# anyboby/Constrained-Model-Based-Policy-Optimization

Measured on AMD Instinct MI355X. Metric: imagined env-steps/sec (ensemble rollout) + CPO update ms, higher is better.
Workload: dtype f32; 1 GPU; AntSafe-v2 imagined rollout: E=7 x (37->512->512->60) swish ensemble, 5 elites, 3+3 critics 128x128, tanh policy 128x128, B=100000 branches/GPU, maxroll 35 (34 steps), fixed-horizon mode, reset->sample*->finish_all_paths->get(); rollout_mode=schedule, branches_per_gpu=100000, branches_total=100000, horizon=34, task=AntSafe-v2

## Files before the change

constrained-model-based-policy-optimization_amd/csrc/ens_h3.hip:

```cpp
#include "common.h"
#include "ens_mlp_internal.h"
#include "f16_split.h"

#include <type_traits>

namespace {

constexpr int kThreadsH = 512;
constexpr int kWavesH = 8;
constexpr int HIDH = 512;

template <int RT>
struct Geo {
  static constexpr int ROWS = 32 * RT;
  static constexpr int NTC = 8 / RT;
  static constexpr int CK = 32 * NTC;
  static constexpr int NCH = HIDH / CK;
  static constexpr int SLC = CK / 32;
  static constexpr int CSTR = CK + 8;
  static constexpr int TPR = kThreadsH / ROWS;
  static constexpr int KPT = 64 / TPR;
  static constexpr int DH = RT == 4 ? 2 : 4;
  static constexpr int NPH = (2 * SLC) % DH == 0 ? 1 : DH;
  static constexpr int CBUF_BYTES = 2 * ROWS * CSTR * 2;
  static constexpr bool W0_LDS = RT == 4;
};

constexpr int PBUF_BYTES = kWavesH * 2 * 16 * 64 * 4;
constexpr int SWS = 65;
constexpr int STG_BYTES = 32 * SWS * 4;
__host__ __device__ constexpr int ximg_bytes(int S0, int RT) { return 2 * 32 * RT * (16 * S0 + 8) * 2; }
__host__ __device__ constexpr int w0buf_bytes(int S0, int RT) { return RT == 4 ? 2 * S0 * 2 * 1024 : 0; }
__host__ __device__ constexpr int off_const(int S0, int RT) {
  const int cb = RT == 4 ? Geo<4>::CBUF_BYTES : (RT == 2 ? Geo<2>::CBUF_BYTES : Geo<1>::CBUF_BYTES);
  const int a = 2 * cb + ximg_bytes(S0, RT) + 2 * w0buf_bytes(S0, RT), b = 2 * PBUF_BYTES + 2 * STG_BYTES;
  return ((a > b ? a : b) + 15) / 16 * 16;
}
constexpr int CONST_FLOATS = 2 * HIDH + 2 * 128 + 6 * 128 + 2 * 64;
__host__ __device__ constexpr int lds_bytes(int S0, int RT) { return off_const(S0, RT) + CONST_FLOATS * 4; }

#ifdef CMBPO_STAMPS
#define H3_STAMP(k)                                                         \
  do {                                                                      \
    __builtin_amdgcn_sched_barrier(0);                                      \
    const unsigned long long t_now = __builtin_amdgcn_s_memtime();          \
    __builtin_amdgcn_s_waitcnt(0xC07F);                                     \
    t_acc[k] += t_now - t_last;                                             \
    t_last = t_now;                                                         \
    __builtin_amdgcn_sched_barrier(0);                                      \
  } while (0)
#else
#define H3_STAMP(k) do { } while (0)
#endif

__global__ void h3_stats_kernel(const float *blob, size_t off0, size_t off1, size_t off2, size_t offb0, size_t offb1, size_t offb2,
                                int kg0, int o_tiles, int hidden, float *stats) {
  const int e = blockIdx.x, l = blockIdx.y, tid = threadIdx.x;
  const int tiles = l == 2 ? o_tiles : hidden / 32, kg = l == 0 ? kg0 : hidden / 8;
  const size_t woff = l == 0 ? off0 : (l == 1 ? off1 : off2), boff = l == 0 ? offb0 : (l == 1 ? offb1 : offb2);
  const float *w = blob + woff + (size_t)e * tiles * kg * 256;
  const float *b = blob + boff + (size_t)e * tiles * 32;
  float wmax = 0.0f, l1 = 0.0f, bmax = 0.0f;
  if (tid < tiles * 32) {
    const int tile = tid >> 5, r = tid & 31;
    for (int g = 0; g < kg; ++g)
      for (int h = 0; h < 2; ++h) {
        const f32x4 v = *reinterpret_cast<const f32x4 *>(w + (((size_t)tile * kg + g) * 64 + h * 32 + r) * 4);
        for (int s = 0; s < 4; ++s) { const float a = fabsf(v[s]); wmax = fmaxf(wmax, a); l1 += a; }
      }
    bmax = fabsf(b[tid]);
  }
  __shared__ float red[3][kThreadsH];
  red[0][tid] = wmax; red[1][tid] = l1; red[2][tid] = bmax;
  __syncthreads();
  for (int st = kThreadsH / 2; st > 0; st >>= 1) {
    if (tid < st)
      for (int q = 0; q < 3; ++q) red[q][tid] = fmaxf(red[q][tid], red[q][tid + st]);
    __syncthreads();
  }
  if (tid == 0) {
    float *o = stats + (size_t)e * NSTAT + 4 * l;
    o[0] = pow2_lift(red[0][0]); o[1] = red[1][0]; o[2] = red[2][0]; o[3] = red[0][0];
  }
}

__global__ void h3_pack_kernel(const float *src, size_t src_stride, int kg, int src_tiles, f16x8 *dst, size_t dst_stride,
                               int n_tiles, int slabs, int members, const float *stats, int layer, int mode) {
  const long idx = (long)blockIdx.x * blockDim.x + threadIdx.x;
  const long per = (long)n_tiles * slabs * 64;
  if (idx >= per * members) return;
  const int e = (int)(idx / per);
  const int rem = (int)(idx - (long)e * per);
  const int lane = rem & 63, s = (rem >> 6) % slabs, tile = (rem >> 6) / slabs;
  const bool m16 = mode >= 2;
  const int n = m16 ? 16 * tile + (lane & 15) : 32 * tile + (lane & 31);
  const int r = n & 31, g = m16 ? lane >> 4 : lane >> 5;
  const float scale = stats[(size_t)e * NSTAT + 4 * layer];
  const float *sp = src + (size_t)e * src_stride;
  f16x8 p1, p2;
#pragma unroll
  for (int j = 0; j < 8; ++j) {
    int k;
    if (mode == 0) k = 16 * s + 8 * g + j;
    else if (mode == 1) {
      const int i = 8 * (s & 1) + j;
      k = 32 * (s >> 1) + (i & 3) + 8 * (i >> 2) + 4 * g;
    } else if (mode == 2) k = 32 * s + 8 * ((g & 1) * 2 + (g >> 1)) + j;
    else k = 32 * s + 16 * (j >> 2) + 4 * g + (j & 3);
    float v = 0.0f;
    if ((n >> 5) < src_tiles && (k >> 3) < kg) v = sp[(((size_t)(n >> 5) * kg + (k >> 3)) * 64 + ((k >> 2) & 1) * 32 + r) * 4 + (k & 3)];
    _Float16 q1, q2;
    split_h(v * scale, q1, q2);
    p1[j] = q1; p2[j] = q2;
  }
  f16x8 *d = dst + (size_t)e * dst_stride + ((size_t)tile * slabs + s) * 2 * 64 + lane;
  d[0] = p1; d[64] = p2;
}

template <int I, int N, class F>
__device__ __forceinline__ void static_for(F &&f) {
  if constexpr (I < N) {
    f(std::integral_constant<int, I>{});
    static_for<I + 1, N>(f);
  }
}


struct H3Args {
  MlpKernelArgs m;
  const f16x8 *w0, *w1, *w2;
  size_t w0_stride, w1_stride, w2_stride;
  const float *stats;
  int item0;
};

template <int S0, int OTP, int RT>
__global__ __launch_bounds__(kThreadsH, 2) void ens_h3_kernel(const H3Args a) {
  using G = Geo<RT>;
  constexpr int ROWSH = G::ROWS, NTC = G::NTC, CK = G::CK, NCH = G::NCH, SLC = G::SLC, CSTR = G::CSTR, TPR = G::TPR,
                KPT = G::KPT, DH = G::DH, NPH = G::NPH, CBUF_BYTES = G::CBUF_BYTES;
  constexpr int XSTR = 16 * S0 + 8;
  constexpr int NPASS = OTP / 2;
  constexpr int NUNIT = RT * NPASS;
  constexpr int O_PAD = 32 * OTP;
  constexpr int W0P = NTC * S0 * 2;
  const MlpKernelArgs &p = a.m;
  extern __shared__ f32x4 smem4[];
  char *smem = reinterpret_cast<char *>(smem4);
  _Float16 *cbuf = reinterpret_cast<_Float16 *>(smem);
  _Float16 *ximg = reinterpret_cast<_Float16 *>(smem + 2 * CBUF_BYTES);
  f16x8 *w0buf = reinterpret_cast<f16x8 *>(smem + 2 * CBUF_BYTES + ximg_bytes(S0, RT));
  f32x4 *pbuf = reinterpret_cast<f32x4 *>(smem);
  float *stg = reinterpret_cast<float *>(smem + 2 * PBUF_BYTES);
  float *cst = reinterpret_cast<float *>(smem + off_const(S0, RT));
  float *bias0 = cst, *bias1 = cst + HIDH, *hc_a = cst + 2 * HIDH, *hc_c = hc_a + 128;
  int *rowidx = reinterpret_cast<int *>(hc_c + 128);
  float *r_inv0 = reinterpret_cast<float *>(rowidx) + 128, *r_t1 = r_inv0 + 128, *r_inv1 = r_t1 + 128, *r_t2 = r_inv1 + 128,
        *r_inv2 = r_t2 + 128;
  float *in_mu_l = r_inv2 + 128, *in_sig_l = in_mu_l + 64;

  const int n_rows = p.n_rows_dev ? *p.n_rows_dev : p.n_rows;
  const int out = p.out_dim;
  if (threadIdx.x < 64) {
    const int k = threadIdx.x;
    in_mu_l[k] = (p.in_mu && k < p.in_dim) ? p.in_mu[k] : 0.0f;
    in_sig_l[k] = (p.in_mu && k < p.in_dim) ? 1.0f / p.in_sig[k] : 1.0f;
  }
  __syncthreads();

  float xpre[KPT];
  float bpre[2], b2pre = 0.0f;
  int rr_pre = -1;
  auto fetch_row = [&](int it, int tid) {
    const int xb = tid / TPR;
    const int e2 = it / p.tiles;
    const int rr = (it - e2 * p.tiles) * ROWSH + xb;
    const bool ok = it < p.n_items && rr < n_rows;
    int v = ok ? rr : 0;
    if (p.row_idx) v = p.row_idx[v];
    rr_pre = ok ? v : -1;
  };
  auto fetch_x = [&](int tid) {
    const int xc = tid % TPR;
    const int rr = rr_pre >= 0 ? rr_pre : 0;
    const float *orow = p.obs + (size_t)rr * p.obs_dim;
    const float *arow = p.act_dim > 0 ? p.act + (size_t)rr * p.act_dim - p.obs_dim : orow;
#pragma unroll
    for (int u = 0; u < KPT; ++u) {
      const int k = KPT * xc + u;
      const float *q = (k < p.obs_dim) ? orow + k : ((k < p.in_dim) ? arow + k : orow);
      xpre[u] = *q;
    }
  };
  auto fetch_bias = [&](int it, int tid) {
    const int e2 = (it < p.n_items) ? it / p.tiles : 0;
    bpre[0] = p.b0[(size_t)e2 * HIDH + tid];
    bpre[1] = p.b1[(size_t)e2 * HIDH + tid];
    const int ob = p.o_tiles * 32;
    b2pre = p.b2[(size_t)e2 * ob + (tid < ob ? tid : 0)];
  };
  fetch_row(a.item0 + blockIdx.x, threadIdx.x);
  fetch_x(threadIdx.x);
  fetch_bias(a.item0 + blockIdx.x, threadIdx.x);
#ifdef CMBPO_STAMPS
  unsigned long long t_acc[12] = {0, 0, 0, 0, 0, 0, 0, 0, 0, 0, 0, 0};
  unsigned long long t_last = __builtin_amdgcn_s_memtime();
  const unsigned long long t_rt0 = __builtin_amdgcn_s_memrealtime();
#endif

  for (int item = a.item0 + blockIdx.x; item < p.n_items; item += gridDim.x) {
    int tid = threadIdx.x;
    asm volatile("v_mov_b32 %0, %0" : "+v"(tid));
    const int lane = tid & 63, wave = __builtin_amdgcn_readfirstlane(tid >> 6);
    const int r = lane & 31, hh = lane >> 5;
    const int xb = tid / TPR, xc = tid % TPR;
    const int e = item / p.tiles;
    const int row0 = (item - e * p.tiles) * ROWSH;
    if (row0 >= n_rows) {
      fetch_row(item + gridDim.x, tid);
      fetch_x(tid);
      fetch_bias(item + gridDim.x, tid);
      continue;
    }
    const float *st = a.stats + (size_t)e * NSTAT;
    const f16x8 *w0e = a.w0 + (size_t)e * a.w0_stride;
    {
      constexpr int W0R = G::W0_LDS ? (2 * W0P + kWavesH - 1) / kWavesH : 1;
      f16x8 w0r[W0R];
      if constexpr (G::W0_LDS) {
#pragma unroll
        for (int u = 0; u < W0R; ++u) {
          const int j = wave + kWavesH * u;
          w0r[u] = w0e[(size_t)(j < 2 * W0P ? j : 0) * 64 + lane];
        }
      }
      bias0[tid] = bpre[0] * kLog2e;
      bias1[tid] = bpre[1] * kLog2e;
      if (tid < O_PAD) {
        float A = 0.0f, Bc = 0.0f;
        if (tid < out) { A = p.out_mu ? p.out_sig[tid] : 1.0f; Bc = p.out_mu ? p.out_mu[tid] : 0.0f; }
        else if (tid < 2 * out) { A = 1.0f; Bc = p.out_mu ? p.out_lsig2[tid - out] : 0.0f; }
        hc_a[tid] = A;
        hc_c[tid] = A * b2pre + Bc;
      }
      float xs[KPT];
      float m = 0.0f;
#pragma unroll
      for (int u = 0; u < KPT; ++u) {
        const int k = KPT * xc + u;
        float x = (xpre[u] - in_mu_l[k & 63]) * in_sig_l[k & 63];
        x = (k < p.in_dim && rr_pre >= 0) ? x : 0.0f;
        xs[u] = x;
        m = fmaxf(m, fabsf(x));
      }
#pragma unroll
      for (int o = 1; o < TPR; o <<= 1) m = fmaxf(m, __shfl_xor(m, o, 64));
      const float t0 = pow2_lift(m);
      if (xc == 0) {
        const float bound1 = (st[1] * m + st[2]) * 1.001f, t1 = pow2_lift(bound1);
        const float bound2 = (st[5] * bound1 + st[6]) * 1.001f, t2 = pow2_lift(bound2);
        rowidx[xb] = rr_pre;
        r_inv0[xb] = 1.0f / (st[0] * t0);
        r_t1[xb] = t1;
        r_inv1[xb] = 1.0f / (st[4] * t1);
        r_t2[xb] = t2;
        r_inv2[xb] = 1.0f / (st[8] * t2);
      }
      if (KPT * xc < 16 * S0) {
        _Float16 q1[KPT], q2[KPT];
#pragma unroll
        for (int u = 0; u < KPT; ++u) split_h(xs[u] * t0, q1[u], q2[u]);
        _Float16 *d1 = ximg + (size_t)xb * XSTR + KPT * xc, *d2 = d1 + (size_t)ROWSH * XSTR;
        if constexpr (KPT >= 8) {
#pragma unroll
          for (int v = 0; v < KPT / 8; ++v) {
            f16x8 w1, w2;
#pragma unroll
            for (int u = 0; u < 8; ++u) { w1[u] = q1[8 * v + u]; w2[u] = q2[8 * v + u]; }
            reinterpret_cast<f16x8 *>(d1)[v] = w1; reinterpret_cast<f16x8 *>(d2)[v] = w2;
          }
        } else {
          f16x4 w1, w2;
#pragma unroll
          for (int u = 0; u < 4; ++u) { w1[u] = q1[u]; w2[u] = q2[u]; }
          *reinterpret_cast<f16x4 *>(d1) = w1; *reinterpret_cast<f16x4 *>(d2) = w2;
        }
      }
      if constexpr (G::W0_LDS) {
#pragma unroll
        for (int u = 0; u < W0R; ++u) {
          const int j = wave + kWavesH * u;
          if (j < 2 * W0P) w0buf[(size_t)j * 64 + lane] = w0r[u];
        }
      }
    }
    fetch_row(item + gridDim.x, tid);
    H3_STAMP(0);
    lds_barrier();
    H3_STAMP(1);

    const int l0_tn = wave & (NTC - 1), l0_bt = wave / NTC;
    const float inv0_l = r_inv0[32 * l0_bt + r] * kLog2e;
    const float t1_l = pow2_rcp(r_t1[32 * l0_bt + r]) * kLog2e;
    const _Float16 *xb0 = ximg + (size_t)(32 * l0_bt + r) * XSTR + 8 * hh;
    struct L0Ops { f16x8 a1, a2, b1, b2; };
    auto l0_read = [&](L0Ops &o, int cc, int s) {
      const f16x8 *wa = G::W0_LDS ? w0buf + ((size_t)(cc & 1) * W0P + (size_t)l0_tn * S0 * 2 + 2 * s) * 64 + lane
                                  : w0e + (((size_t)(cc < NCH ? cc : NCH - 1) * NTC + l0_tn) * S0 * 2 + 2 * s) * 64 + lane;
      o.a1 = wa[0]; o.a2 = wa[64];
      o.b1 = *reinterpret_cast<const f16x8 *>(xb0 + 16 * s);
      o.b2 = *reinterpret_cast<const f16x8 *>(xb0 + (size_t)ROWSH * XSTR + 16 * s);
    };
    auto l0_store = [&](const Epi4 &s, int cc, int q) {
      _Float16 *c1 = cbuf + (size_t)(cc & 1) * (CBUF_BYTES / 2) + (size_t)(32 * l0_bt + r) * CSTR + 32 * l0_tn + 4 * hh + 8 * q;
      *reinterpret_cast<uint2 *>(c1) = make_uint2(s.q1[0], s.q1[1]);
      *reinterpret_cast<uint2 *>(c1 + (size_t)ROWSH * CSTR) = make_uint2(s.q2[0], s.q2[1]);
    };
    auto l0_bias = [&](int cc, int q) {
      return *reinterpret_cast<const f32x4 *>(bias0 + cc * CK + 32 * l0_tn + 8 * q + 4 * hh);
    };

    constexpr int VT = 2 * RT;
    const int c16 = lane & 15, g4 = lane >> 4;
    const int sig = c16 < 4 ? 2 * c16 : (c16 < 12 ? 2 * c16 - 7 : 2 * c16 - 16);
    const int pik = 8 * (2 * (g4 & 1) + (g4 >> 1));
    f32x4 acc[4][VT];
#pragma unroll
    for (int u = 0; u < 4; ++u)
#pragma unroll
      for (int v = 0; v < VT; ++v)
#pragma unroll
        for (int i = 0; i < 4; ++i) acc[u][v][i] = 0.0f;
    const f16x8 *w1a = a.w1 + (size_t)e * a.w1_stride + (size_t)(4 * wave) * 16 * 128 + lane;
    f16x8 A[DH][2][2];
    f16x8 Bt[2][2];
    auto load_h = [&](f16x8 (&x)[2][2], int h) {
      h = h < 31 ? h : 31;
#pragma unroll
      for (int t = 0; t < 2; ++t) {
        const f16x8 *q = w1a + ((size_t)(2 * (h & 1) + t) * 16 + (h >> 1)) * 128;
        x[t][0] = q[0]; x[t][1] = q[64];
      }
    };
    auto read_b = [&](f16x8 (&x)[2], const _Float16 *img, int v, int sl) {
      const _Float16 *q = img + (size_t)(16 * v + sig) * CSTR + 32 * sl + pik;
      x[0] = *reinterpret_cast<const f16x8 *>(q);
      x[1] = *reinterpret_cast<const f16x8 *>(q + (size_t)ROWSH * CSTR);
    };
#pragma unroll
    for (int h = 0; h < DH; ++h) load_h(A[h], h);
    {
      f32x16 d;
#pragma unroll
      for (int i = 0; i < 16; ++i) d[i] = 0.0f;
#pragma unroll
      for (int s = 0; s < S0; ++s) {
        L0Ops o;
        l0_read(o, 0, s);
        mm3(d, o.a1, o.a2, o.b1, o.b2);
      }
#pragma unroll
      for (int q = 0; q < 4; ++q) {
        Epi4 es;
        const f32x4 bv = l0_bias(0, q);
        epi_all<false>(es, d, q, inv0_l, bv, t1_l);
        l0_store(es, 0, q);
      }
    }
    lds_barrier();
    H3_STAMP(2);

    auto step = [&](auto LASTC, const int c, auto PHC) {
      constexpr bool LAST = decltype(LASTC)::value;
      constexpr int PH = decltype(PHC)::value;
      f16x8 wst;
      const bool stage_w0 = c + 2 < NCH;
      const int cw = stage_w0 ? c + 2 : NCH - 1;
      const _Float16 *img = cbuf + (size_t)(c & 1) * (CBUF_BYTES / 2);
      f32x16 d;
#pragma unroll
      for (int i = 0; i < 16; ++i) d[i] = 0.0f;
      L0Ops l0;
      Epi4 es;
      f32x4 bv = {0.0f, 0.0f, 0.0f, 0.0f};
      read_b(Bt[0], img, 0, 0);
      if constexpr (!LAST) l0_read(l0, c + 1, 0);
#pragma unroll
      for (int slot = 0; slot < 8; ++slot) {
        if (!LAST && slot >= 4) bv = l0_bias(c + 1, slot - 4);
        if constexpr (G::W0_LDS && !LAST) {
          if (slot == 4) wst = w0e[((size_t)cw * W0P + wave) * 64 + lane];
          if (slot == 5 && W0P > kWavesH) {
            if (stage_w0) w0buf[((size_t)(c & 1) * W0P + wave) * 64 + lane] = wst;
            wst = w0e[((size_t)cw * W0P + (wave + kWavesH < W0P ? wave + kWavesH : wave)) * 64 + lane];
          }
        }
#pragma unroll
        for (int i = 0; i < 24; ++i) {
          const int pos = 2 * slot + i / 12;
          const int sl = pos / VT, v = pos % VT;
          const int u = (i % 12) / 3, term = i % 3;
          const int hl = 2 * sl + (u >> 1);
          f16x8(&Ah)[2][2] = A[(PH * 2 * SLC + hl) % DH];
          if (i % 12 == 0) {
            if (pos + 1 < 16) read_b(Bt[(pos + 1) & 1], img, (pos + 1) % VT, (pos + 1) / VT);
            if (i == 0) __builtin_amdgcn_sched_barrier(0);
          }
          f32x4 &ac = acc[u][v];
          const f16x8 &b1 = Bt[pos & 1][0], &b2 = Bt[pos & 1][1];
          if (term == 0) ac = __builtin_amdgcn_mfma_f32_16x16x32_f16(Ah[u & 1][1], b1, ac, 0, 0, 0);
          else if (term == 1) ac = __builtin_amdgcn_mfma_f32_16x16x32_f16(Ah[u & 1][0], b2, ac, 0, 0, 0);
          else ac = __builtin_amdgcn_mfma_f32_16x16x32_f16(Ah[u & 1][0], b1, ac, 0, 0, 0);
          if (v == VT - 1 && (i % 12 == 5 || i % 12 == 11) && !(LAST && hl + DH >= 2 * SLC))
            load_h(Ah, c * 2 * SLC + hl + DH);
          if (!LAST && slot < S0 && i == 11) {
            mm3(d, l0.a1, l0.a2, l0.b1, l0.b2);
            if (slot + 1 < S0) l0_read(l0, c + 1, slot + 1);
          }
          if (!LAST && slot >= 4 && i % 2 == 0) {
            const int q = slot - 4, k = i / 2;
            if (k == 0) epi_stage<0, true>(es, d, q, inv0_l, bv, t1_l);
            if (k == 2) epi_stage<2, true>(es, d, q, inv0_l, bv, t1_l);
            if (k == 3) epi_stage<3, true>(es, d, q, inv0_l, bv, t1_l);
            if (k == 4) epi_stage<4, true>(es, d, q, inv0_l, bv, t1_l);
            if (k == 5) epi_stage<5, true>(es, d, q, inv0_l, bv, t1_l);
            if (k == 6) epi_stage<6, true>(es, d, q, inv0_l, bv, t1_l);
            if (k == 8) epi_stage<8, true>(es, d, q, inv0_l, bv, t1_l);
            if (k == 9) epi_stage<9, true>(es, d, q, inv0_l, bv, t1_l);
            if (k == 10) l0_store(es, c + 1, q);
          }
          __builtin_amdgcn_sched_barrier(0);
        }
      }
      H3_STAMP(4);
      if constexpr (G::W0_LDS && !LAST) {
        if (stage_w0) {
          const int j = W0P > kWavesH ? wave + kWavesH : wave;
          if (j < W0P) w0buf[((size_t)(c & 1) * W0P + j) * 64 + lane] = wst;
        }
      }
      lds_barrier();
      H3_STAMP(5);
    };
    {
      constexpr int NREG = NCH - 1, NFULL = NREG / NPH * NPH;
#pragma unroll 1
      for (int c0 = 0; c0 < NFULL; c0 += NPH)
        static_for<0, NPH>([&](auto P) { step(std::false_type{}, c0 + decltype(P)::value, P); });
      static_for<0, NREG - NFULL>([&](auto P) { step(std::false_type{}, NFULL + decltype(P)::value, P); });
      step(std::true_type{}, NREG, std::integral_constant<int, NREG % NPH>{});
    }

    fetch_x(tid);
    fetch_bias(item + gridDim.x, tid);
    H3_STAMP(6);

    const f16x8 *w2w = a.w2 + (size_t)e * a.w2_stride + lane;
    auto reduce_unit = [&](int u) {
      const int rt = u / NPASS, pass = u % NPASS;
      const int tt = wave >> 2, q = wave & 3;
      const f32x4 *pp = pbuf + ((size_t)(u & 1) * 64 + (size_t)tt * 4 + q) * 64 + lane;
      f32x4 v = pp[0];
#pragma unroll
      for (int wv = 1; wv < kWavesH; ++wv) v += pp[(size_t)wv * 8 * 64];
      const int nl = 32 * tt + 8 * q + 4 * hh, n = 64 * pass + nl;
      const f32x4 ha = *reinterpret_cast<const f32x4 *>(hc_a + n), hc = *reinterpret_cast<const f32x4 *>(hc_c + n);
      const float inv2_l = r_inv2[32 * rt + r];
      float *sg = stg + (size_t)(u & 1) * 32 * SWS + r * SWS + nl;
#pragma unroll
      for (int s = 0; s < 4; ++s) {
        float y = ha[s] * (v[s] * inv2_l) + hc[s];
        if (n + s >= out) y = __expf(y);
        sg[s] = y;
      }
    };
    auto store_unit = [&](int u) {
      const int rt = u / NPASS, pass = u % NPASS;
      if (NPASS == 1 && (out & 1) == 0) {
        const int half = lane >= out ? 1 : 0, c = 2 * (lane - half * out);
#pragma unroll
        for (int j = 0; j < 2; ++j) {
          const int rl = wave + kWavesH * (2 * j + half);
          const int rr = rowidx[32 * rt + rl];
          const float *sp = stg + (size_t)(u & 1) * 32 * SWS + rl * SWS + c;
          const float2 y = make_float2(sp[0], sp[1]);
          if (rr >= 0 && lane < 2 * out) {
            const size_t obase = ((size_t)e * p.ld_rows + rr) * out;
            float *dst = c < out ? p.out0 + obase + c : p.out1 + obase + (c - out);
            *reinterpret_cast<float2 *>(dst) = y;
          }
        }
        return;
      }
      const int n = 64 * pass + lane;
#pragma unroll
      for (int j = 0; j < 4; ++j) {
        const int rl = wave + kWavesH * j;
        const int rr = rowidx[32 * rt + rl];
        const float y = stg[(size_t)(u & 1) * 32 * SWS + rl * SWS + lane];
        if (rr >= 0 && n < 2 * out) {
          const size_t obase = ((size_t)e * p.ld_rows + rr) * out;
          if (n < out) p.out0[obase + n] = y;
          else p.out1[obase + (n - out)] = y;
        }
      }
    };
    auto h2_frag = [&](u32x4 (&bfu)[2][2][2], auto RTI) {
      constexpr int rt = decltype(RTI)::value;
#pragma unroll
      for (int vv = 0; vv < 2; ++vv) {
        const int row = 32 * rt + 16 * vv + sig;
        const float inv1_l = r_inv1[row] * kLog2e;
        const float t2_l = pow2_rcp(r_t2[row]) * kLog2e;
#pragma unroll
        for (int u = 0; u < 4; ++u) {
          const f32x4 bv = *reinterpret_cast<const f32x4 *>(bias1 + 64 * wave + 16 * u + 4 * g4);
          Epi4 es;
          epi_all<false>(es, acc[u][2 * rt + vv], 0, inv1_l, bv, t2_l);
          bfu[vv][u >> 1][0][2 * (u & 1)] = es.q1[0]; bfu[vv][u >> 1][0][2 * (u & 1) + 1] = es.q1[1];
          bfu[vv][u >> 1][1][2 * (u & 1)] = es.q2[0]; bfu[vv][u >> 1][1][2 * (u & 1) + 1] = es.q2[1];
        }
      }
    };
    auto out_mm = [&](f32x4 (&o)[2][2], const f16x8 (&w)[2][2], const u32x4 (&bfu)[2][2][2], int ks) {
#pragma unroll
      for (int vv = 0; vv < 2; ++vv) {
        const f16x8 b1 = __builtin_bit_cast(f16x8, bfu[vv][ks][0]), b2 = __builtin_bit_cast(f16x8, bfu[vv][ks][1]);
#pragma unroll
        for (int aa = 0; aa < 2; ++aa) mm3(o[aa][vv], w[aa][0], w[aa][1], b1, b2);
      }
    };
    auto put_partials = [&](const f32x4 (&o)[2][2][2], int u) {
      f32x4 *pw = pbuf + ((size_t)(u & 1) * 64 + (size_t)wave * 8) * 64;
#pragma unroll
      for (int tt = 0; tt < 2; ++tt)
#pragma unroll
        for (int aa = 0; aa < 2; ++aa)
#pragma unroll
          for (int vv = 0; vv < 2; ++vv)
            pw[(size_t)(tt * 4 + 2 * aa + (g4 >> 1)) * 64 + 16 * vv + sig + 32 * (g4 & 1)] = o[tt][aa][vv];
    };
    auto zero_o = [&](f32x4 (&o)[2][2][2]) {
#pragma unroll
      for (int tt = 0; tt < 2; ++tt)
#pragma unroll
        for (int aa = 0; aa < 2; ++aa)
#pragma unroll
          for (int vv = 0; vv < 2; ++vv)
#pragma unroll
            for (int i = 0; i < 4; ++i) o[tt][aa][vv][i] = 0.0f;
    };
    if constexpr (NPASS == 1) {
      f16x8 w2r[2][2][2][2];
#pragma unroll
      for (int ks = 0; ks < 2; ++ks)
#pragma unroll
        for (int ot = 0; ot < 4; ++ot) {
          const f16x8 *q = w2w + ((size_t)ot * 16 + 2 * wave + ks) * 128;
          w2r[ks][ot >> 1][ot & 1][0] = q[0]; w2r[ks][ot >> 1][ot & 1][1] = q[64];
        }
      u32x4 bfu[2][2][2][2];
      auto stA = [&](auto RTI) { h2_frag(bfu[decltype(RTI)::value & 1], RTI); };
      auto stB = [&](auto RTI) {
        constexpr int rt = decltype(RTI)::value;
        f32x4 o[2][2][2];
        zero_o(o);
#pragma unroll
        for (int ks = 0; ks < 2; ++ks)
#pragma unroll
          for (int tt = 0; tt < 2; ++tt) out_mm(o[tt], w2r[ks][tt], bfu[rt & 1], ks);
        put_partials(o, rt);
      };
      stA(std::integral_constant<int, 0>{});
      static_for<0, RT + 2>([&](auto KI) {
        constexpr int k = decltype(KI)::value;
        if constexpr (k >= 2 && k - 2 < RT) store_unit(k - 2);
        if constexpr (k >= 1 && k - 1 < RT) reduce_unit(k - 1);
        if constexpr (k < RT) stB(std::integral_constant<int, (k < RT ? k : 0)>{});
        if constexpr (k + 1 < RT) stA(std::integral_constant<int, (k + 1 < RT ? k + 1 : 0)>{});
        H3_STAMP(7);
        if constexpr (k + 1 < RT + 2) lds_barrier();
        H3_STAMP(8);
      });
    } else {
      static_for<0, RT>([&](auto RTI) {
        constexpr int rt = decltype(RTI)::value;
        f16x8 wf[2][2][2];
        auto load_w2 = [&](f16x8 (&x)[2][2], int pass, int st) {
#pragma unroll
          for (int aa = 0; aa < 2; ++aa) {
            const f16x8 *q = w2w + ((size_t)(4 * pass + 2 * (st & 1) + aa) * 16 + 2 * wave + (st >> 1)) * 128;
            x[aa][0] = q[0]; x[aa][1] = q[64];
          }
        };
        load_w2(wf[0], 0, 0);
        u32x4 bfu[2][2][2];
        h2_frag(bfu, RTI);
#pragma unroll
        for (int pass = 0; pass < NPASS; ++pass) {
          const int u = rt * NPASS + pass;
          f32x4 o[2][2][2];
          zero_o(o);
#pragma unroll
          for (int st = 0; st < 4; ++st) {
            if (st < 3 || pass + 1 < NPASS) load_w2(wf[(st & 1) ^ 1], st == 3 ? pass + 1 : pass, (st + 1) & 3);
            out_mm(o[st & 1], wf[st & 1], bfu, st >> 1);
          }
          put_partials(o, u);
          H3_STAMP(7);
          lds_barrier();
          H3_STAMP(8);
          if (u > 0) store_unit(u - 1);
          reduce_unit(u);
          H3_STAMP(9);
        }
      });
      lds_barrier();
      store_unit(NUNIT - 1);
    }
    H3_STAMP(10);
    lds_barrier();
    H3_STAMP(11);
  }
#ifdef CMBPO_STAMPS
  if (p.stamps && threadIdx.x == 0) {
    for (int k = 0; k < 12; ++k) p.stamps[(size_t)blockIdx.x * 16 + k] = t_acc[k];
    p.stamps[(size_t)blockIdx.x * 16 + 12] = __builtin_amdgcn_s_memrealtime() - t_rt0;
  }
#endif
}

}

static int ensure_h3(cmbpo_mlp *m, hipStream_t s) {
  const int H = m->hidden, E = m->ensemble;
  const int S0 = m->h3_s0, OTP = m->h3_otp;
  const int slabs[3] = {S0, H / 32, H / 32};
  const int tiles[3] = {H / 32, H / 16, 2 * OTP};
  if (m->d_h3 == nullptr) {
    size_t off = 0;
    for (int l = 0; l < 3; ++l) {
      m->h3_stride[l] = (size_t)tiles[l] * slabs[l] * 2 * 64;
      m->h3_off[l] = off;
      off += m->h3_stride[l] * E;
    }
    m->h3_stats_off = off;
    const size_t bytes = off * 16 + (size_t)E * NSTAT * sizeof(float);
    if (hipMalloc(&m->d_h3, bytes) != hipSuccess) {
      (void)hipGetLastError();
      m->d_h3 = nullptr;
      cmbpo_set_error("ens_h3: hipMalloc of the f16 weight images failed");
      return CMBPO_ENOMEM;
    }
    m->h3_version = ~0ul;
  }
  if (m->h3_version == m->pack_version) return CMBPO_OK;
  float *stats = reinterpret_cast<float *>(reinterpret_cast<char *>(m->d_h3) + m->h3_stats_off * 16);
  hipLaunchKernelGGL(h3_stats_kernel, dim3(E, 3), dim3(kThreadsH), 0, s, m->d_blob, m->off_wp0, m->off_wp1, m->off_wp2,
                     m->off_b0, m->off_b1, m->off_b2, m->in_pad / 8, m->o_tiles, H, stats);
  const size_t src_off[3] = {m->off_wp0, m->off_wp1, m->off_wp2};
  const int kg[3] = {m->in_pad / 8, H / 8, H / 8};
  const int src_tiles[3] = {H / 32, H / 32, m->o_tiles};
  for (int l = 0; l < 3; ++l) {
    const size_t src_stride = (size_t)src_tiles[l] * kg[l] * 256;
    const long total = (long)tiles[l] * slabs[l] * 64 * E;
    hipLaunchKernelGGL(h3_pack_kernel, dim3((unsigned)((total + 255) / 256)), dim3(256), 0, s, m->d_blob + src_off[l], src_stride,
                       kg[l], src_tiles[l], reinterpret_cast<f16x8 *>(m->d_h3) + m->h3_off[l], m->h3_stride[l], tiles[l], slabs[l],
                       E, stats, l, l == 0 ? 0 : l + 1);
  }
  CMBPO_HIP_CHECK(hipGetLastError());
  m->h3_version = m->pack_version;
  return CMBPO_OK;
}

void cmbpo_internal_f16_stats(const cmbpo_mlp *m, float *stats, hipStream_t s) {
  hipLaunchKernelGGL(h3_stats_kernel, dim3(m->ensemble, 3), dim3(kThreadsH), 0, s, m->d_blob, m->off_wp0, m->off_wp1, m->off_wp2,
                     m->off_b0, m->off_b1, m->off_b2, m->in_pad / 8, m->o_tiles, m->hidden, stats);
}
void cmbpo_internal_f16_pack(const cmbpo_mlp *m, int layer, void *dst, size_t dst_stride, int n_tiles, int slabs, int perm,
                             const float *stats, hipStream_t s) {
  const int H = m->hidden;
  const size_t src_off[3] = {m->off_wp0, m->off_wp1, m->off_wp2};
  const int kg[3] = {m->in_pad / 8, H / 8, H / 8};
  const int src_tiles[3] = {H / 32, H / 32, m->o_tiles};
  const size_t src_stride = (size_t)src_tiles[layer] * kg[layer] * 256;
  const long total = (long)n_tiles * slabs * 64 * m->ensemble;
  hipLaunchKernelGGL(h3_pack_kernel, dim3((unsigned)((total + 255) / 256)), dim3(256), 0, s, m->d_blob + src_off[layer], src_stride,
                     kg[layer], src_tiles[layer], reinterpret_cast<f16x8 *>(dst), dst_stride, n_tiles, slabs, m->ensemble, stats, layer,
                     perm);
}

static int g_h3_rt = 0;
extern "C" int cmbpo_set_ens_f16_row_tiles(int rt) {
  CMBPO_REQUIRE(rt == 0 || rt == 1 || rt == 2 || rt == 4, "cmbpo_set_ens_f16_row_tiles: 0 (by row count), 1, 2 or 4");
  g_h3_rt = rt;
  return CMBPO_OK;
}

bool cmbpo_internal_h3_eligible(const cmbpo_mlp *m) {
  return m->head == CMBPO_HEAD_PROB && m->hidden == 512 && m->act == CMBPO_ACT_SWISH && m->o_tiles <= 4 && m->in_pad <= 64 &&
         2 * m->out_dim == m->o_width;
}

int cmbpo_internal_launch_h3(cmbpo_mlp *m, MlpKernelArgs &a, hipStream_t s) {
  if (m->h3_s0 == 0) {
    const int s0 = (m->in_pad + 15) / 16;
    m->h3_s0 = s0 < 2 ? 2 : s0;
    m->h3_otp = m->o_tiles <= 2 ? 2 : 4;
  }
  if (int rc = ensure_h3(m, s)) return rc;
  H3Args k{};
  k.m = a;
  const f16x8 *base = reinterpret_cast<const f16x8 *>(m->d_h3);
  k.w0 = base + m->h3_off[0]; k.w1 = base + m->h3_off[1]; k.w2 = base + m->h3_off[2];
  k.w0_stride = m->h3_stride[0]; k.w1_stride = m->h3_stride[1]; k.w2_stride = m->h3_stride[2];
  k.stats = reinterpret_cast<const float *>(reinterpret_cast<const char *>(m->d_h3) + m->h3_stats_off * 16);
  const int n_cu = cmbpo_cu_count();
  const int E = m->ensemble;
  constexpr int kSplitGap = 40;
  int RT = g_h3_rt, RT_tail = 0, full = 0, tail_start = 0;
  if (RT == 0) {
    const int first_two[3] = {220, 310, 550}, steady_two[3] = {175, 300, 540};
    const int first_four[3] = {255, 360, 720}, steady_four[3] = {198, 343, 705};
    const int *first = m->h3_otp > 2 ? first_four : first_two, *steady = m->h3_otp > 2 ? steady_four : steady_two;
    const int rts[3] = {1, 2, 4};
    auto cost_of = [&](int i, long rounds) -> long { return rounds <= 0 ? 0 : first[i] + (rounds - 1) * steady[i]; };
    long best = -1;
    for (int i = 0; i < 3; ++i) {
      const long cost = cost_of(i, cmbpo_ceil_div(cmbpo_ceil_div(a.n_rows, 32 * rts[i]) * E, n_cu));
      if (best < 0 || cost <= best) { best = cost; RT = rts[i]; }
    }
    for (int i = 1; i < 3; ++i) {
      const int tiles_m = cmbpo_ceil_div(a.n_rows, 32 * rts[i]), n_m = tiles_m * E;
      const int fl = n_m / n_cu * n_cu, left = n_m - fl;
      if (fl == 0 || left == 0) continue;
      const int e0 = fl / tiles_m, t0 = fl - e0 * tiles_m;
      for (int j = 0; j < i; ++j) {
        const int tiles_t = cmbpo_ceil_div(a.n_rows, 32 * rts[j]);
        const int start = e0 * tiles_t + (rts[i] / rts[j]) * t0, n_tail = tiles_t * E - start;
        const long cost = cost_of(i, fl / n_cu) + cost_of(j, cmbpo_ceil_div(n_tail, n_cu)) + kSplitGap;
        if (cost < best) { best = cost; RT = rts[i]; RT_tail = rts[j]; full = fl; tail_start = start; }
      }
    }
  }
  const int S0 = m->h3_s0, OTP = m->h3_otp;
  auto launch = [&](int rt, int item0, int end) -> int {
    const int tiles = cmbpo_ceil_div(a.n_rows, 32 * rt);
    k.m.tiles = tiles;
    k.m.n_items = end < 0 ? tiles * E : end;
    k.item0 = item0;
    const size_t lds = (size_t)lds_bytes(S0, rt);
    CMBPO_REQUIRE(lds <= 160 * 1024, "ens_h3: LDS budget exceeded (%zu B)", lds);
    const int n_here = k.m.n_items - item0;
    const int grid = n_here < n_cu ? n_here : n_cu;
#define CMBPO_H3_CASE(S0_, OTP_, RT_)                                                                                  \
  if (S0 == S0_ && OTP == OTP_ && rt == RT_) {                                                                         \
    if (int rc = cmbpo_grant_lds(ens_h3_kernel<S0_, OTP_, RT_>, lds)) return rc;                                      \
    hipLaunchKernelGGL((ens_h3_kernel<S0_, OTP_, RT_>), dim3(grid), dim3(kThreadsH), lds, s, k);                      \
  }
#define CMBPO_H3_CASES(RT_)                                                                                            \
  CMBPO_H3_CASE(2, 2, RT_) CMBPO_H3_CASE(3, 2, RT_) CMBPO_H3_CASE(4, 2, RT_)                                           \
  CMBPO_H3_CASE(2, 4, RT_) CMBPO_H3_CASE(3, 4, RT_) CMBPO_H3_CASE(4, 4, RT_)
    CMBPO_H3_CASES(4) CMBPO_H3_CASES(2) CMBPO_H3_CASES(1)
#undef CMBPO_H3_CASES
#undef CMBPO_H3_CASE
    CMBPO_HIP_CHECK(hipGetLastError());
    return CMBPO_OK;
  };
  if (RT_tail) {
    if (int rc = launch(RT, 0, full)) return rc;
    return launch(RT_tail, tail_start, -1);
  }
  return launch(RT, 0, -1);
}
```

Baseline: 67.07 million imagined env-steps/s.

## Stage next item's inputs and constants during the last layer-1 step

Splits the per-item prologue (input fetch, normalisation, f16 split, bias/head constants, W0 staging to LDS) into 24 small pieces. Those pieces are interleaved into the final hidden-layer step of the current item and write into a double-buffered constant region, so the next item's prologue overlaps with MFMA work instead of running serially before the barrier. To fit the second constant buffer in LDS, the partial-sum buffer is single-buffered, which adds extra barriers in the output layer. Dead items are skipped ahead of time via next_alive. The risks are higher register pressure from the StageRegs state and the added output-stage synchronisation.

```diff
diff --git a/constrained-model-based-policy-optimization_amd/csrc/ens_h3.hip b/constrained-model-based-policy-optimization_amd/csrc/ens_h3.hip
--- a/constrained-model-based-policy-optimization_amd/csrc/ens_h3.hip
+++ b/constrained-model-based-policy-optimization_amd/csrc/ens_h3.hip
@@ -29,15 +29,25 @@
 constexpr int PBUF_BYTES = kWavesH * 2 * 16 * 64 * 4;
 constexpr int SWS = 65;
 constexpr int STG_BYTES = 32 * SWS * 4;
+__host__ __device__ constexpr bool stage_ahead(int S0, int RT) { return !(S0 == 4 && RT == 4); }
+__host__ __device__ constexpr int tail_bytes(int S0, int RT) { return (stage_ahead(S0, RT) ? 1 : 2) * PBUF_BYTES + 2 * STG_BYTES; }
 __host__ __device__ constexpr int ximg_bytes(int S0, int RT) { return 2 * 32 * RT * (16 * S0 + 8) * 2; }
 __host__ __device__ constexpr int w0buf_bytes(int S0, int RT) { return RT == 4 ? 2 * S0 * 2 * 1024 : 0; }
+__host__ __device__ constexpr int r16(int v) { return (v + 15) / 16 * 16; }
+__host__ __device__ constexpr int off_ximg(int S0, int RT) {
+  const int cb = 2 * (RT == 4 ? Geo<4>::CBUF_BYTES : (RT == 2 ? Geo<2>::CBUF_BYTES : Geo<1>::CBUF_BYTES));
+  return stage_ahead(S0, RT) && tail_bytes(S0, RT) > cb ? r16(tail_bytes(S0, RT)) : cb;
+}
 __host__ __device__ constexpr int off_const(int S0, int RT) {
-  const int cb = RT == 4 ? Geo<4>::CBUF_BYTES : (RT == 2 ? Geo<2>::CBUF_BYTES : Geo<1>::CBUF_BYTES);
-  const int a = 2 * cb + ximg_bytes(S0, RT) + 2 * w0buf_bytes(S0, RT), b = 2 * PBUF_BYTES + 2 * STG_BYTES;
-  return ((a > b ? a : b) + 15) / 16 * 16;
-}
-constexpr int CONST_FLOATS = 2 * HIDH + 2 * 128 + 6 * 128 + 2 * 64;
-__host__ __device__ constexpr int lds_bytes(int S0, int RT) { return off_const(S0, RT) + CONST_FLOATS * 4; }
+  const int a = off_ximg(S0, RT) + ximg_bytes(S0, RT) + 2 * w0buf_bytes(S0, RT);
+  return r16(a > tail_bytes(S0, RT) ? a : tail_bytes(S0, RT));
+}
+constexpr int ITEM_FLOATS = 2 * HIDH + 2 * 128 + 6 * 128;
+__host__ __device__ constexpr int lds_bytes(int S0, int RT) {
+  return off_const(S0, RT) + ((stage_ahead(S0, RT) ? 2 : 1) * ITEM_FLOATS + 2 * 64) * 4;
+}
+static_assert(lds_bytes(4, 4) == 156416 && lds_bytes(3, 4) == 152320 && lds_bytes(2, 4) <= 160 * 1024 &&
+              lds_bytes(4, 2) <= 160 * 1024 && lds_bytes(4, 1) <= 160 * 1024, "ens_h3: LDS map");
 
 #ifdef CMBPO_STAMPS
 #define H3_STAMP(k)                                                         \
@@ -126,6 +136,20 @@
 }
 
 
+constexpr int kPieces = 24, kReqEarly = 5;
+__host__ __device__ constexpr int piece_at(int slot, int i) {
+  if (i % 2 != 0) return -1;
+  const int k = i / 2;
+  if (slot == 0) return k % 3 == 0 ? k / 3 : -1;
+  if (slot == 1) return k == 0 ? 4 : (k == 2 ? 5 : (k == 4 ? 6 : -1));
+  if (slot == 3) return k == 4 ? 13 : -1;
+  if (slot == 4) return k == 1 ? 7 : -1;
+  if (slot == 5) return k == 4 ? 20 : (k >= 6 && k < 10 ? 2 + k : -1);
+  if (slot == 6) return k == 0 ? 12 : (k == 1 ? 14 : (k == 3 ? 15 : (k == 5 ? 16 : (k >= 7 && k <= 9 ? 10 + k : (k == 10 ? 21 : -1)))));
+  if (slot == 7) return k < 2 ? 22 + k : -1;
+  return -1;
+}
+
 struct H3Args {
   MlpKernelArgs m;
   const f16x8 *w0, *w1, *w2;
@@ -144,20 +168,26 @@
   constexpr int NUNIT = RT * NPASS;
   constexpr int O_PAD = 32 * OTP;
   constexpr int W0P = NTC * S0 * 2;
+  constexpr bool AHEAD = stage_ahead(S0, RT);
   const MlpKernelArgs &p = a.m;
   extern __shared__ f32x4 smem4[];
   char *smem = reinterpret_cast<char *>(smem4);
   _Float16 *cbuf = reinterpret_cast<_Float16 *>(smem);
-  _Float16 *ximg = reinterpret_cast<_Float16 *>(smem + 2 * CBUF_BYTES);
-  f16x8 *w0buf = reinterpret_cast<f16x8 *>(smem + 2 * CBUF_BYTES + ximg_bytes(S0, RT));
+  _Float16 *ximg = reinterpret_cast<_Float16 *>(smem + off_ximg(S0, RT));
+  f16x8 *w0buf = reinterpret_cast<f16x8 *>(smem + off_ximg(S0, RT) + ximg_bytes(S0, RT));
+  constexpr bool PB2 = !AHEAD;
   f32x4 *pbuf = reinterpret_cast<f32x4 *>(smem);
-  float *stg = reinterpret_cast<float *>(smem + 2 * PBUF_BYTES);
+  float *stg = reinterpret_cast<float *>(smem + (PB2 ? 2 : 1) * PBUF_BYTES);
   float *cst = reinterpret_cast<float *>(smem + off_const(S0, RT));
-  float *bias0 = cst, *bias1 = cst + HIDH, *hc_a = cst + 2 * HIDH, *hc_c = hc_a + 128;
-  int *rowidx = reinterpret_cast<int *>(hc_c + 128);
-  float *r_inv0 = reinterpret_cast<float *>(rowidx) + 128, *r_t1 = r_inv0 + 128, *r_inv1 = r_t1 + 128, *r_t2 = r_inv1 + 128,
-        *r_inv2 = r_t2 + 128;
-  float *in_mu_l = r_inv2 + 128, *in_sig_l = in_mu_l + 64;
+  struct Cst { float *bias0, *bias1, *hc_a, *hc_c; int *rowidx; float *r_inv0, *r_t1, *r_inv1, *r_t2, *r_inv2; };
+  auto cst_of = [&](int par) {
+    Cst c;
+    c.bias0 = cst + (AHEAD ? par : 0) * ITEM_FLOATS; c.bias1 = c.bias0 + HIDH; c.hc_a = c.bias0 + 2 * HIDH; c.hc_c = c.hc_a + 128;
+    c.rowidx = reinterpret_cast<int *>(c.hc_c + 128);
+    c.r_inv0 = c.hc_c + 256; c.r_t1 = c.r_inv0 + 128; c.r_inv1 = c.r_t1 + 128; c.r_t2 = c.r_inv1 + 128; c.r_inv2 = c.r_t2 + 128;
+    return c;
+  };
+  float *in_mu_l = cst + (AHEAD ? 2 : 1) * ITEM_FLOATS, *in_sig_l = in_mu_l + 64;
 
   const int n_rows = p.n_rows_dev ? *p.n_rows_dev : p.n_rows;
   const int out = p.out_dim;
@@ -168,8 +198,14 @@
   }
   __syncthreads();
 
-  float xpre[KPT];
-  float bpre[2], b2pre = 0.0f;
+  auto next_alive = [&](int it) {
+    while (it < p.n_items) {
+      const int e2 = it / p.tiles;
+      if ((it - e2 * p.tiles) * ROWSH < n_rows) break;
+      it += gridDim.x;
+    }
+    return it;
+  };
   int rr_pre = -1;
   auto fetch_row = [&](int it, int tid) {
     const int xb = tid / TPR;
@@ -180,124 +216,177 @@
     if (p.row_idx) v = p.row_idx[v];
     rr_pre = ok ? v : -1;
   };
-  auto fetch_x = [&](int tid) {
-    const int xc = tid % TPR;
-    const int rr = rr_pre >= 0 ? rr_pre : 0;
-    const float *orow = p.obs + (size_t)rr * p.obs_dim;
-    const float *arow = p.act_dim > 0 ? p.act + (size_t)rr * p.act_dim - p.obs_dim : orow;
-#pragma unroll
-    for (int u = 0; u < KPT; ++u) {
-      const int k = KPT * xc + u;
-      const float *q = (k < p.obs_dim) ? orow + k : ((k < p.in_dim) ? arow + k : orow);
-      xpre[u] = *q;
-    }
+
+  constexpr int W0R = G::W0_LDS ? (2 * W0P + kWavesH - 1) / kWavesH : 1;
+  constexpr int GQ = KPT / 4;
+  struct StageRegs {
+    float x[KPT];
+    float b0, b1, b2, hs, hm, hl;
+    float st[7];
+    f16x8 w0r[W0R];
+    float m, t0, t1, t2;
+    unsigned q1[KPT / 2], q2[KPT / 2];
   };
-  auto fetch_bias = [&](int it, int tid) {
-    const int e2 = (it < p.n_items) ? it / p.tiles : 0;
-    bpre[0] = p.b0[(size_t)e2 * HIDH + tid];
-    bpre[1] = p.b1[(size_t)e2 * HIDH + tid];
-    const int ob = p.o_tiles * 32;
-    b2pre = p.b2[(size_t)e2 * ob + (tid < ob ? tid : 0)];
+  auto stage_piece = [&](auto KC, auto FRONTC, StageRegs &s, const int es, const Cst &c, const int tid, const int it_next) {
+    constexpr int K = decltype(KC)::value;
+    constexpr bool FRONT = decltype(FRONTC)::value;
+    const int xb = tid / TPR, xc = tid % TPR;
+    if constexpr (K < 4) {
+      const int rr = rr_pre >= 0 ? rr_pre : 0;
+      const float *orow = p.obs + (size_t)rr * p.obs_dim;
+      const float *arow = p.act_dim > 0 ? p.act + (size_t)rr * p.act_dim - p.obs_dim : orow;
+#pragma unroll
+      for (int u = GQ * K; u < GQ * K + GQ; ++u) {
+        const int k = KPT * xc + u;
+        const bool in_obs = k < p.obs_dim, in_act = !in_obs & (k < p.in_dim);
+        const float *base = in_act ? arow : orow;
+        const int off = (in_obs | in_act) ? k : 0;
+        s.x[u] = base[off];
+      }
+    } else if constexpr (K == 4) {
+      s.b0 = p.b0[(size_t)es * HIDH + tid];
+      s.b1 = p.b1[(size_t)es * HIDH + tid];
+      const int ob = p.o_tiles * 32;
+      s.b2 = p.b2[(size_t)es * ob + (tid < ob ? tid : 0)];
+    } else if constexpr (K == 5) {
+      s.hs = 1.0f; s.hm = 0.0f; s.hl = 0.0f;
+      if (p.out_mu) {
+        const int ia = tid < out ? tid : out - 1, il = tid < out ? 0 : (tid < 2 * out ? tid - out : out - 1);
+        s.hs = p.out_sig[ia]; s.hm = p.out_mu[ia]; s.hl = p.out_lsig2[il];
+      }
+      const float *st = a.stats + (size_t)es * NSTAT;
+      s.st[0] = st[0]; s.st[1] = st[1]; s.st[2] = st[2]; s.st[3] = st[4]; s.st[4] = st[5]; s.st[5] = st[6]; s.st[6] = st[8];
+    } else if constexpr (K == 6 || K == 13 || K == 20 || K == 22) {
+      if constexpr (G::W0_LDS) {
+        const int lane = tid & 63, wave = __builtin_amdgcn_readfirstlane(tid >> 6);
+        const f16x8 *w0s = a.w0 + (size_t)es * a.w0_stride;
+        auto get = [&](f16x8 &x, int u) { const int j = wave + kWavesH * u; x = w0s[(size_t)(j < 2 * W0P ? j : 0) * 64 + lane]; };
+        auto put = [&](const f16x8 &x, int u) { const int j = wave + kWavesH * u; if (j < 2 * W0P) w0buf[(size_t)j * 64 + lane] = x; };
+        if constexpr (FRONT) {
+#pragma unroll
+          for (int u = 0; u < W0R; ++u) {
+            if constexpr (K == 6) get(s.w0r[u], u);
+            if constexpr (K == 22) put(s.w0r[u], u);
+          }
+        } else {
+          constexpr int u = K == 6 ? 0 : (K == 13 ? 1 : (K == 20 ? 2 : 3));
+          static_assert(W0R <= 3, "ens_h3: rounds of the W0 chunks");
+          if constexpr (u >= 1 && u <= W0R) put(s.w0r[0], u - 1);
+          if constexpr (u < W0R) get(s.w0r[0], u);
+        }
+      }
+    } else if constexpr (K == 7) {
+      c.bias0[tid] = s.b0 * kLog2e;
+      c.bias1[tid] = s.b1 * kLog2e;
+      if (tid < O_PAD) {
+        const bool is_mean = tid < out, is_var = !is_mean & (tid < 2 * out);
+        float A = is_var ? 1.0f : 0.0f, Bc = is_var ? s.hl : 0.0f;
+        A = is_mean ? s.hs : A; Bc = is_mean ? s.hm : Bc;
+        c.hc_a[tid] = A;
+        c.hc_c[tid] = A * s.b2 + Bc;
+      }
+    } else if constexpr (K < 12) {
+      if constexpr (K == 8) s.m = 0.0f;
+#pragma unroll
+      for (int u = GQ * (K - 8); u < GQ * (K - 8) + GQ; ++u) {
+        const int k = KPT * xc + u;
+        float x = (s.x[u] - in_mu_l[k & 63]) * in_sig_l[k & 63];
+        const bool keep = (k < p.in_dim) & (rr_pre >= 0);
+        x = keep ? x : 0.0f;
+        s.x[u] = x;
+        s.m = fmaxf(s.m, fabsf(x));
+        asm volatile("" : "+v"(s.x[u]));
+      }
+      asm volatile("" : "+v"(s.m));
+    } else if constexpr (K == 12) {
+#pragma unroll
+      for (int o = 1; o < TPR; o <<= 1) s.m = fmaxf(s.m, __shfl_xor(s.m, o, 64));
+      s.t0 = pow2_lift(s.m);
+      asm volatile("" : "+v"(s.m), "+v"(s.t0));
+    } else if constexpr (K == 14) {
+      if (xc == 0) {
+        const float bound1 = (s.st[1] * s.m + s.st[2]) * 1.001f, t1 = pow2_lift(bound1);
+        const float bound2 = (s.st[4] * bound1 + s.st[5]) * 1.001f, t2 = pow2_lift(bound2);
+        c.rowidx[xb] = rr_pre;
+        c.r_inv0[xb] = 1.0f / (s.st[0] * s.t0);
+        c.r_t1[xb] = t1;
+        c.r_t2[xb] = t2;
+        s.t1 = t1; s.t2 = t2;
+      }
+    } else if constexpr (K == 15) {
+      if (xc == 0) {
+        c.r_inv1[xb] = 1.0f / (s.st[3] * s.t1);
+        c.r_inv2[xb] = 1.0f / (s.st[6] * s.t2);
+      }
+    } else if constexpr (K < 20) {
+#pragma unroll
+      for (int u = GQ * (K - 16); u < GQ * (K - 16) + GQ; ++u) {
+        _Float16 h1, h2;
+        split_h(s.x[u] * s.t0, h1, h2);
+        if (u % 2 == 0) { s.q1[u / 2] = __builtin_bit_cast(unsigned short, h1); s.q2[u / 2] = __builtin_bit_cast(unsigned short, h2); }
+        else {
+          s.q1[u / 2] |= (unsigned)__builtin_bit_cast(unsigned short, h1) << 16;
+          s.q2[u / 2] |= (unsigned)__builtin_bit_cast(unsigned short, h2) << 16;
+          asm volatile("" : "+v"(s.q1[u / 2]), "+v"(s.q2[u / 2]));
+        }
+      }
+    } else if constexpr (K == 21) {
+      if (KPT * xc < 16 * S0) {
+        _Float16 *d1 = ximg + (size_t)xb * XSTR + KPT * xc, *d2 = d1 + (size_t)ROWSH * XSTR;
+        if constexpr (KPT >= 8) {
+#pragma unroll
+          for (int v = 0; v < KPT / 8; ++v) {
+            u32x4 w1, w2;
+#pragma unroll
+            for (int u = 0; u < 4; ++u) { w1[u] = s.q1[4 * v + u]; w2[u] = s.q2[4 * v + u]; }
+            reinterpret_cast<u32x4 *>(d1)[v] = w1; reinterpret_cast<u32x4 *>(d2)[v] = w2;
+          }
+        } else {
+          *reinterpret_cast<uint2 *>(d1) = make_uint2(s.q1[0], s.q1[1]);
+          *reinterpret_cast<uint2 *>(d2) = make_uint2(s.q2[0], s.q2[1]);
+        }
+      }
+    } else {
+      fetch_row(it_next, tid);
+    }
   };
-  fetch_row(a.item0 + blockIdx.x, threadIdx.x);
-  fetch_x(threadIdx.x);
-  fetch_bias(a.item0 + blockIdx.x, threadIdx.x);
 #ifdef CMBPO_STAMPS
   unsigned long long t_acc[12] = {0, 0, 0, 0, 0, 0, 0, 0, 0, 0, 0, 0};
   unsigned long long t_last = __builtin_amdgcn_s_memtime();
   const unsigned long long t_rt0 = __builtin_amdgcn_s_memrealtime();
 #endif
 
-  for (int item = a.item0 + blockIdx.x; item < p.n_items; item += gridDim.x) {
+  StageRegs sr;
+  auto stage_front = [&](int es, const Cst &c, int tid, int it_next) {
+    static_for<kReqEarly, kPieces>([&](auto P) { stage_piece(P, std::true_type{}, sr, es, c, tid, it_next); });
+    H3_STAMP(0);
+    lds_barrier();
+    H3_STAMP(1);
+  };
+  int item = next_alive(a.item0 + blockIdx.x);
+  int nxt = next_alive(item + gridDim.x);
+  int par = 0;
+  if (item < p.n_items) {
+    fetch_row(item, threadIdx.x);
+    const int e0 = item / p.tiles;
+    static_for<0, kReqEarly>([&](auto P) { stage_piece(P, std::true_type{}, sr, e0, cst_of(0), threadIdx.x, 0); });
+    if constexpr (AHEAD) stage_front(e0, cst_of(0), threadIdx.x, nxt);
+  }
+
+  while (item < p.n_items) {
     int tid = threadIdx.x;
     asm volatile("v_mov_b32 %0, %0" : "+v"(tid));
     const int lane = tid & 63, wave = __builtin_amdgcn_readfirstlane(tid >> 6);
     const int r = lane & 31, hh = lane >> 5;
-    const int xb = tid / TPR, xc = tid % TPR;
     const int e = item / p.tiles;
-    const int row0 = (item - e * p.tiles) * ROWSH;
-    if (row0 >= n_rows) {
-      fetch_row(item + gridDim.x, tid);
-      fetch_x(tid);
-      fetch_bias(item + gridDim.x, tid);
-      continue;
-    }
-    const float *st = a.stats + (size_t)e * NSTAT;
+    const int e_nxt = (nxt < p.n_items ? nxt : item) / p.tiles;
+    const int nxt2 = next_alive(nxt + gridDim.x);
+    const Cst cc = cst_of(par);
+    float *const bias0 = cc.bias0, *const bias1 = cc.bias1, *const hc_a = cc.hc_a, *const hc_c = cc.hc_c;
+    int *const rowidx = cc.rowidx;
+    float *const r_inv0 = cc.r_inv0, *const r_t1 = cc.r_t1, *const r_inv1 = cc.r_inv1, *const r_t2 = cc.r_t2, *const r_inv2 = cc.r_inv2;
     const f16x8 *w0e = a.w0 + (size_t)e * a.w0_stride;
-    {
-      constexpr int W0R = G::W0_LDS ? (2 * W0P + kWavesH - 1) / kWavesH : 1;
-      f16x8 w0r[W0R];
-      if constexpr (G::W0_LDS) {
-#pragma unroll
-        for (int u = 0; u < W0R; ++u) {
-          const int j = wave + kWavesH * u;
-          w0r[u] = w0e[(size_t)(j < 2 * W0P ? j : 0) * 64 + lane];
-        }
-      }
-      bias0[tid] = bpre[0] * kLog2e;
-      bias1[tid] = bpre[1] * kLog2e;
-      if (tid < O_PAD) {
-        float A = 0.0f, Bc = 0.0f;
-        if (tid < out) { A = p.out_mu ? p.out_sig[tid] : 1.0f; Bc = p.out_mu ? p.out_mu[tid] : 0.0f; }
-        else if (tid < 2 * out) { A = 1.0f; Bc = p.out_mu ? p.out_lsig2[tid - out] : 0.0f; }
-        hc_a[tid] = A;
-        hc_c[tid] = A * b2pre + Bc;
-      }
-      float xs[KPT];
-      float m = 0.0f;
-#pragma unroll
-      for (int u = 0; u < KPT; ++u) {
-        const int k = KPT * xc + u;
-        float x = (xpre[u] - in_mu_l[k & 63]) * in_sig_l[k & 63];
-        x = (k < p.in_dim && rr_pre >= 0) ? x : 0.0f;
-        xs[u] = x;
-        m = fmaxf(m, fabsf(x));
-      }
-#pragma unroll
-      for (int o = 1; o < TPR; o <<= 1) m = fmaxf(m, __shfl_xor(m, o, 64));
-      const float t0 = pow2_lift(m);
-      if (xc == 0) {
-        const float bound1 = (st[1] * m + st[2]) * 1.001f, t1 = pow2_lift(bound1);
-        const float bound2 = (st[5] * bound1 + st[6]) * 1.001f, t2 = pow2_lift(bound2);
-        rowidx[xb] = rr_pre;
-        r_inv0[xb] = 1.0f / (st[0] * t0);
-        r_t1[xb] = t1;
-        r_inv1[xb] = 1.0f / (st[4] * t1);
-        r_t2[xb] = t2;
-        r_inv2[xb] = 1.0f / (st[8] * t2);
-      }
-      if (KPT * xc < 16 * S0) {
-        _Float16 q1[KPT], q2[KPT];
-#pragma unroll
-        for (int u = 0; u < KPT; ++u) split_h(xs[u] * t0, q1[u], q2[u]);
-        _Float16 *d1 = ximg + (size_t)xb * XSTR + KPT * xc, *d2 = d1 + (size_t)ROWSH * XSTR;
-        if constexpr (KPT >= 8) {
-#pragma unroll
-          for (int v = 0; v < KPT / 8; ++v) {
-            f16x8 w1, w2;
-#pragma unroll
-            for (int u = 0; u < 8; ++u) { w1[u] = q1[8 * v + u]; w2[u] = q2[8 * v + u]; }
-            reinterpret_cast<f16x8 *>(d1)[v] = w1; reinterpret_cast<f16x8 *>(d2)[v] = w2;
-          }
-        } else {
-          f16x4 w1, w2;
-#pragma unroll
-          for (int u = 0; u < 4; ++u) { w1[u] = q1[u]; w2[u] = q2[u]; }
-          *reinterpret_cast<f16x4 *>(d1) = w1; *reinterpret_cast<f16x4 *>(d2) = w2;
-        }
-      }
-      if constexpr (G::W0_LDS) {
-#pragma unroll
-        for (int u = 0; u < W0R; ++u) {
-          const int j = wave + kWavesH * u;
-          if (j < 2 * W0P) w0buf[(size_t)j * 64 + lane] = w0r[u];
-        }
-      }
-    }
-    fetch_row(item + gridDim.x, tid);
-    H3_STAMP(0);
-    lds_barrier();
-    H3_STAMP(1);
+    if constexpr (!AHEAD) stage_front(e, cc, tid, nxt);
 
     const int l0_tn = wave & (NTC - 1), l0_bt = wave / NTC;
     const float inv0_l = r_inv0[32 * l0_bt + r] * kLog2e;
@@ -373,6 +462,15 @@
     auto step = [&](auto LASTC, const int c, auto PHC) {
       constexpr bool LAST = decltype(LASTC)::value;
       constexpr int PH = decltype(PHC)::value;
+      constexpr bool STG = LAST && AHEAD;
+      const bool have_next = nxt < p.n_items;
+      StageRegs sa;
+      int tid_s = 0;
+      if constexpr (STG) {
+        tid_s = threadIdx.x;
+        asm volatile("v_mov_b32 %0, %0" : "+v"(tid_s));
+      }
+      const Cst cn = cst_of(par ^ 1);
       f16x8 wst;
       const bool stage_w0 = c + 2 < NCH;
       const int cw = stage_w0 ? c + 2 : NCH - 1;
@@ -385,8 +483,8 @@
       f32x4 bv = {0.0f, 0.0f, 0.0f, 0.0f};
       read_b(Bt[0], img, 0, 0);
       if constexpr (!LAST) l0_read(l0, c + 1, 0);
-#pragma unroll
-      for (int slot = 0; slot < 8; ++slot) {
+      static_for<0, 8>([&](auto SLOTC) {
+        constexpr int slot = decltype(SLOTC)::value;
         if (!LAST && slot >= 4) bv = l0_bias(c + 1, slot - 4);
         if constexpr (G::W0_LDS && !LAST) {
           if (slot == 4) wst = w0e[((size_t)cw * W0P + wave) * 64 + lane];
@@ -395,8 +493,8 @@
             wst = w0e[((size_t)cw * W0P + (wave + kWavesH < W0P ? wave + kWavesH : wave)) * 64 + lane];
           }
         }
-#pragma unroll
-        for (int i = 0; i < 24; ++i) {
+        static_for<0, 24>([&](auto IC) {
+          constexpr int i = decltype(IC)::value;
           const int pos = 2 * slot + i / 12;
           const int sl = pos / VT, v = pos % VT;
           const int u = (i % 12) / 3, term = i % 3;
@@ -429,8 +527,17 @@
             if (k == 9) epi_stage<9, true>(es, d, q, inv0_l, bv, t1_l);
             if (k == 10) l0_store(es, c + 1, q);
           }
+          if constexpr (STG && piece_at(slot, i) >= 0)
+            if (have_next) stage_piece(std::integral_constant<int, (piece_at(slot, i) >= 0 ? piece_at(slot, i) : 0)>{}, std::false_type{}, sa, e_nxt, cn, tid_s, nxt2);
           __builtin_amdgcn_sched_barrier(0);
-        }
+        });
+      });
+      if constexpr (STG) {
+        static_for<0, 24>([&](auto IC) {
+          constexpr int pc = piece_at(8, decltype(IC)::value);
+          if constexpr (pc >= 0)
+            if (have_next) stage_piece(std::integral_constant<int, (pc >= 0 ? pc : 0)>{}, std::false_type{}, sa, e_nxt, cn, tid_s, nxt2);
+        });
       }
       H3_STAMP(4);
       if constexpr (G::W0_LDS && !LAST) {
@@ -450,16 +557,16 @@
       static_for<0, NREG - NFULL>([&](auto P) { step(std::false_type{}, NFULL + decltype(P)::value, P); });
       step(std::true_type{}, NREG, std::integral_constant<int, NREG % NPH>{});
     }
-
-    fetch_x(tid);
-    fetch_bias(item + gridDim.x, tid);
+    if constexpr (!AHEAD) {
+      if (nxt < p.n_items) static_for<0, kReqEarly>([&](auto P) { stage_piece(P, std::true_type{}, sr, e_nxt, cc, tid, 0); });
+    }
     H3_STAMP(6);
 
     const f16x8 *w2w = a.w2 + (size_t)e * a.w2_stride + lane;
     auto reduce_unit = [&](int u) {
       const int rt = u / NPASS, pass = u % NPASS;
       const int tt = wave >> 2, q = wave & 3;
-      const f32x4 *pp = pbuf + ((size_t)(u & 1) * 64 + (size_t)tt * 4 + q) * 64 + lane;
+      const f32x4 *pp = pbuf + ((size_t)(PB2 ? u & 1 : 0) * 64 + (size_t)tt * 4 + q) * 64 + lane;
       f32x4 v = pp[0];
 #pragma unroll
       for (int wv = 1; wv < kWavesH; ++wv) v += pp[(size_t)wv * 8 * 64];
@@ -531,7 +638,7 @@
       }
     };
     auto put_partials = [&](const f32x4 (&o)[2][2][2], int u) {
-      f32x4 *pw = pbuf + ((size_t)(u & 1) * 64 + (size_t)wave * 8) * 64;
+      f32x4 *pw = pbuf + ((size_t)(PB2 ? u & 1 : 0) * 64 + (size_t)wave * 8) * 64;
 #pragma unroll
       for (int tt = 0; tt < 2; ++tt)
 #pragma unroll
@@ -569,6 +676,7 @@
         for (int ks = 0; ks < 2; ++ks)
 #pragma unroll
           for (int tt = 0; tt < 2; ++tt) out_mm(o[tt], w2r[ks][tt], bfu[rt & 1], ks);
+        if (!PB2 && rt > 0) lds_barrier();
         put_partials(o, rt);
       };
       stA(std::integral_constant<int, 0>{});
@@ -606,6 +714,7 @@
             if (st < 3 || pass + 1 < NPASS) load_w2(wf[(st & 1) ^ 1], st == 3 ? pass + 1 : pass, (st + 1) & 3);
             out_mm(o[st & 1], wf[st & 1], bfu, st >> 1);
           }
+          if (!PB2 && u > 0) lds_barrier();
           put_partials(o, u);
           H3_STAMP(7);
           lds_barrier();
@@ -621,6 +730,7 @@
     H3_STAMP(10);
     lds_barrier();
     H3_STAMP(11);
+    item = nxt; nxt = nxt2; par ^= 1;
   }
 #ifdef CMBPO_STAMPS
   if (p.stamps && threadIdx.x == 0) {
```

Result: faster. 68.05 million imagined env-steps/s (median of 6 runs) (+1.5%).
